# GPUs/goVideoCompressor

Hardware: AMD Instinct MI355X
Metric: encoded frames/sec (whole node), 1080p30->H.264 CRF23 (higher is better)
Workload: dtype uint8 (8-bit 4:2:0 samples, int32 transforms)

## Files before the change

csrc/kernels/encode_inter.hip:

```cpp
#include "h264_trellis.h"
#include "mb_row.h"

namespace mivc {
namespace gpu {

using h264::MbHeader;

struct InterArgs {
  Geom g;
  const uint8_t *src_y, *src_u, *src_v;
  const uint8_t *ref_y, *ref_u, *ref_v;
  uint8_t *rec_y, *rec_u, *rec_v;
  const uint8_t* pred_y;
  const int16_t* mv;
  const int16_t* mv8;
  const int* me_cost;
  const int* intra_cost;
  const int* qp;
  const int8_t* aq;
  int chroma_qp_offset;
  MbHeader* hdr;
  int16_t* coef;
  uint8_t* nz;
  uint8_t* intra_flag;
  int* intra_count;
  const uint8_t *ref1_u, *ref1_v;
  int bmode;
  int w1[4];
  int t8;
  const uint8_t* refs_u[4];
  const uint8_t* refs_v[4];
  const int8_t* mref;
  const int* wp;
  int trellis;
  float trellis_lambda;
  const SlotRoute* rt;
  int nbuf;
  uint8_t* qp_flags;
};


__device__ __forceinline__ int wp_sample(int p, int w, int o, int d) {
  return h264::clip1((d >= 1 ? ((p * w + (1 << (d - 1))) >> d) : p * w) + o);
}


__device__ __forceinline__ void chroma_mc4x4(const uint8_t* refc, int cw, int CH, int px0, int py0, int mvx, int mvy,
                                             int (&pv)[4][4]) {
  const int xf = mvx & 7, yf = mvy & 7;
  const int xi = px0 + (mvx >> 3), yi = py0 + (mvy >> 3);
  int rw[5][5];
  if (xi >= 0 && xi + 8 <= cw && yi >= 0 && yi + 5 <= CH) {
#pragma unroll
    for (int r = 0; r < 5; ++r) {
      const uint8_t* row = refc + static_cast<size_t>(yi + r) * cw;
      const int a = xi & ~3;
      const uint32_t w0 = *reinterpret_cast<const uint32_t*>(row + a), w1 = *reinterpret_cast<const uint32_t*>(row + a + 4);
      const uint32_t w4 = __builtin_amdgcn_alignbyte(w1, w0, xi & 3), w5 = row[xi + 4];
#pragma unroll
      for (int c = 0; c < 4; ++c) rw[r][c] = __builtin_amdgcn_ubfe(w4, 8 * c, 8);
      rw[r][4] = w5;
    }
  } else {
#pragma unroll
    for (int r = 0; r < 5; ++r) {
      const uint8_t* row = refc + static_cast<size_t>(clampi(yi + r, 0, CH - 1)) * cw;
#pragma unroll
      for (int c = 0; c < 5; ++c) rw[r][c] = row[clampi(xi + c, 0, cw - 1)];
    }
  }
  const int wA = (8 - xf) * (8 - yf), wB = xf * (8 - yf), wC = (8 - xf) * yf, wD = xf * yf;
#pragma unroll
  for (int y = 0; y < 4; ++y)
#pragma unroll
    for (int x = 0; x < 4; ++x)
      pv[y][x] = (wA * rw[y][x] + wB * rw[y][x + 1] + wC * rw[y + 1][x] + wD * rw[y + 1][x + 1] + 32) >> 6;
}

__device__ __forceinline__ int decimate_score(const int* scan, int start) {
  int score = 0, last = start - 1;
  bool big = false;
#pragma unroll
  for (int i = 0; i < 16; ++i) {
    if (i < start) continue;
    const int v = scan[i];
    const bool nzv = v != 0;
    big |= v > 1 || v < -1;
    const int run = i - last - 1;
    const int t = run == 0 ? 3 : (run <= 2 ? 2 : (run <= 5 ? 1 : 0));
    score += nzv ? t : 0;
    last = nzv ? i : last;
  }
  return big ? 9 : score;
}

__device__ __forceinline__ uint32_t ld4(const uint8_t* row, int x) {
  const int a = x & ~3;
  const uint32_t w0 = *reinterpret_cast<const uint32_t*>(row + a), w1 = *reinterpret_cast<const uint32_t*>(row + a + 4);
  return __builtin_amdgcn_alignbyte(w1, w0, x & 3);
}

__global__ __launch_bounds__(64) __attribute__((amdgpu_waves_per_eu(4, 8))) void encode_inter_mb(InterArgs a) {
  const Geom& g = a.g;
  const int lane = threadIdx.x, q = lane >> 4, l = lane & 15;
  const int nmb = g.nmb();
  int ux, slot;
  xcd_unit_slot(ux, slot);
  if (!route_active(a.rt, slot, a.bmode ? SK_B : SK_P)) return;
  const size_t rcur = route_index(a.rt, a.nbuf, slot, RO_CUR);
  const int W = g.W, cw = g.cw(), CH = g.ch();
  const int mb0 = ux * kMbsPerWave, mx0 = mb0 % g.wmb, my0 = mb0 / g.wmb;
  auto locate = [&](int qi, int& mx, int& my, size_t& o, bool& work, int& qp) {
    const bool live = mb0 + qi < nmb;
    const int d = live ? qi : nmb - 1 - mb0;
    mx = mx0 + d;
    my = my0;
#pragma unroll
    for (int i = 0; i < 3; ++i) {
      const bool wrap = mx >= g.wmb;
      mx -= wrap ? g.wmb : 0;
      my += wrap ? 1 : 0;
    }
    o = static_cast<size_t>(slot) * nmb + mb0 + d;
    work = live && !(a.intra_cost[o] < a.me_cost[o]);
    qp = clampi(a.qp[slot] + (a.aq ? a.aq[o] : 0), 0, 51);
    return live;
  };

  __shared__ uint32_t s_px[kMbsPerWave][2][16][4];
  __shared__ int s_d8[kMbsPerWave][4][64];

  auto store_levels = [](int16_t* dst, const int* v) {
    uint32_t w[8];
#pragma unroll
    for (int i = 0; i < 8; ++i) w[i] = (static_cast<uint32_t>(v[2 * i]) & 0xFFFFu) | (static_cast<uint32_t>(v[2 * i + 1]) << 16);
    reinterpret_cast<uint4*>(dst)[0] = make_uint4(w[0], w[1], w[2], w[3]);
    reinterpret_cast<uint4*>(dst)[1] = make_uint4(w[4], w[5], w[6], w[7]);
  };

  int lv[16];
  int res[16];
  uint32_t prw[4];
  uint64_t luma_any = 0;

  {
    int mx, my, qp;
    size_t o;
    bool work;
    const bool live = locate(q, mx, my, o, work, qp);
    MbHeader* h = a.hdr + o;
    int16_t* coef = a.coef + o * h264::kCoefPerMb;
    if (live && !work && l == 0) {
      a.intra_flag[o] = 1;
      atomicAdd(a.intra_count + slot, 1);
      h->kind = h264::MBK_I16x16;
    }
    const int X0 = mx * 16, Y0 = my * 16;
    const int lbx = (((l >> 2) & 1) * 2 + (l & 1)) * 4, lby = (((l >> 3) & 1) * 2 + ((l >> 1) & 1)) * 4;
    const int k = l & 3, ox = lbx & 4, oy = lby & 4;
    int* dd = s_d8[q][l >> 2];

    int score = 0;
    if (work) {
      const uint8_t* srcy = a.src_y + slot * g.ysize() + static_cast<size_t>(Y0 + lby) * W + X0 + lbx;
      const uint8_t* pred = a.pred_y + o * 256 + lby * 16 + lbx;
      uint32_t sw[4];
#pragma unroll
      for (int y = 0; y < 4; ++y) {
        prw[y] = *reinterpret_cast<const uint32_t*>(pred + y * 16);
        sw[y] = *reinterpret_cast<const uint32_t*>(srcy + static_cast<size_t>(y) * W);
      }
      if (a.wp && !a.bmode && !(a.mref && a.mref[o])) {
        const int* wt = a.wp + slot * 8;
        const int w = wt[0], wo = wt[1], d = wt[2];
        if (w != (1 << d) || wo != 0) {
#pragma unroll
          for (int y = 0; y < 4; ++y) {
            int v4[4];
#pragma unroll
            for (int x = 0; x < 4; ++x) v4[x] = wp_sample(static_cast<int>(__builtin_amdgcn_ubfe(prw[y], 8 * x, 8)), w, wo, d);
            prw[y] = pack4_u8(v4);
          }
        }
      }
#pragma unroll
      for (int y = 0; y < 4; ++y)
#pragma unroll
        for (int x = 0; x < 4; ++x)
          res[y * 4 + x] = static_cast<int>(__builtin_amdgcn_ubfe(sw[y], 8 * x, 8)) -
                           static_cast<int>(__builtin_amdgcn_ubfe(prw[y], 8 * x, 8));
      h264::forward_core4x4(res);
      int mf[3];
#pragma unroll
      for (int c = 0; c < 3; ++c) mf[c] = h264::kQuantMF[qp % 6][c];
      const int qbits = 15 + qp / 6;
      if (a.trellis) {
        trellis_lite4x4(res, lv, mf, qbits, trellis_lambda4(a.trellis_lambda, qp));
      } else {
#pragma unroll
        for (int r = 0; r < 16; ++r) lv[r] = h264::quant_coef(res[r], mf[h264::kPosClass[r]], qbits, 11);
      }
      int scan[16];
#pragma unroll
      for (int i = 0; i < 16; ++i) scan[i] = lv[h264::kZigzag4x4[i]];
      score = decimate_score(scan, 0);
      if (a.t8) {
#pragma unroll
        for (int y = 0; y < 4; ++y) {
          s_px[q][0][lby + y][lbx >> 2] = sw[y];
          s_px[q][1][lby + y][lbx >> 2] = prw[y];
        }
      }
    }
    const int score8 = sum4(score), score16 = sum16(score);
    const bool keep4 = score8 >= 4 && score16 >= 6;

    bool use8 = false, keep8 = false;
    uint64_t use8_wave = 0;
    if (a.t8) {
      wave_sync();
      const uint64_t try_wave = __ballot(keep4);
      if (try_wave) {
        const bool mine = ((try_wave >> (16 * q)) & 0xFFFFu) != 0;
        int satd = 0;
        if (mine) {
          int r2[16];
#pragma unroll
          for (int y = 0; y < 4; ++y) {
            const uint32_t sv = s_px[q][0][lby + y][lbx >> 2], pv = s_px[q][1][lby + y][lbx >> 2];
#pragma unroll
            for (int x = 0; x < 4; ++x) {
              r2[y * 4 + x] = static_cast<int>(__builtin_amdgcn_ubfe(sv, 8 * x, 8)) -
                              static_cast<int>(__builtin_amdgcn_ubfe(pv, 8 * x, 8));
              dd[(oy + y) * 8 + ox + x] = r2[y * 4 + x];
            }
          }
          satd = h264::satd4x4(r2);
        }
        const int col = l, grp = q;
        mfma_i32x4 sop, pop;
        {
          const int cm = col >> 2, b8 = col & 3, r0 = (b8 >> 1) * 8 + 2 * grp, c0 = (b8 & 1) * 2;
#pragma unroll
          for (int sp = 0; sp < 2; ++sp) {
            mfma_i32x4& op = sp ? pop : sop;
            op[0] = static_cast<int>(s_px[cm][sp][r0][c0] ^ 0x80808080u);
            op[1] = static_cast<int>(s_px[cm][sp][r0][c0 + 1] ^ 0x80808080u);
            op[2] = static_cast<int>(s_px[cm][sp][r0 + 1][c0] ^ 0x80808080u);
            op[3] = static_cast<int>(s_px[cm][sp][r0 + 1][c0 + 1] ^ 0x80808080u);
          }
        }
        mfma_i32x4 hp, hn;
#pragma unroll
        for (int j = 0; j < 4; ++j) {
          uint32_t w = 0;
#pragma unroll
          for (int b = 0; b < 4; ++b) w |= ((__builtin_popcount(col & (4 * j + b)) & 1) ? 0xFFu : 0x01u) << (8 * b);
          hp[j] = static_cast<int>(w);
          hn[j] = static_cast<int>(w ^ 0xFEFEFEFEu);
        }
        int sa = 0;
#pragma unroll
        for (int t = 0; t < 4; ++t) {
          const bool neg = __builtin_popcount(t & grp) & 1;
          mfma_i32x4 d = __builtin_amdgcn_mfma_i32_16x16x64_i8(neg ? hn : hp, sop, mfma_i32x4{0, 0, 0, 0}, 0, 0, 0);
          d = __builtin_amdgcn_mfma_i32_16x16x64_i8(neg ? hp : hn, pop, d, 0, 0, 0);
          sa += abs(d[0]) + abs(d[1]) + abs(d[2]) + abs(d[3]);
        }
        sa = sum_row_groups(sa);
        const int sa8d = __shfl(sum4((sa + 2) >> 2), 4 * q, 64);
        const int satd16 = sum16(satd);
        use8 = mine && sa8d < satd16;
        use8_wave = __ballot(use8);
        wave_sync();
        if (use8_wave) {
          if (use8) {
            dct8_pass(dd + (2 * k) * 8, 1);
            dct8_pass(dd + (2 * k + 1) * 8, 1);
          }
          wave_sync();
          if (use8) {
            dct8_pass(dd + 2 * k, 8);
            dct8_pass(dd + 2 * k + 1, 8);
          }
          wave_sync();
          const int qbits8 = 16 + qp / 6;
          const int m = qp % 6;
          if (a.trellis >= 2) {
            float z[16];
            int nzc = 0;
            if (use8) {
              const float inv = exp2f(-static_cast<float>(qbits8));
#pragma unroll
              for (int i = 0; i < 16; ++i) {
                const int pos = kZz8[k * 16 + i];
                const int mf8 = kQuant8MF[m][pos8(pos & 7, pos >> 3)];
                z[i] = static_cast<float>(dd[pos]) * static_cast<float>(mf8) * inv;
                nzc |= h264::quant_coef(dd[pos], mf8, qbits8, 11) != 0;
              }
            }
            const int nz1 = quad_bcast<1>(nzc), nz2 = quad_bcast<2>(nzc), nz3 = quad_bcast<3>(nzc);
            const bool later = (k < 1 && nz1) || (k < 2 && nz2) || (k < 3 && nz3);
            if (use8) trellis_lite8_chunk(z, lv, a.trellis_lambda * 0.136f, later);
          } else if (use8) {
#pragma unroll
            for (int i = 0; i < 16; ++i) {
              const int pos = kZz8[k * 16 + i];
              lv[i] = h264::quant_coef(dd[pos], kQuant8MF[m][pos8(pos & 7, pos >> 3)], qbits8, 11);
            }
          }
          int lastnz = -1, firstnz = -1, inner = 0, big = 0;
          if (use8) {
#pragma unroll
            for (int i = 0; i < 16; ++i) {
              const int idx = k * 16 + i;
              const int v = lv[i];
              const bool nzv = v != 0;
              big |= v > 1 || v < -1;
              const int run = idx - lastnz - 1;
              inner += (nzv && firstnz >= 0) ? (run <= 3 ? 3 : (run <= 11 ? 2 : (run <= 23 ? 1 : 0))) : 0;
              firstnz = (nzv && firstnz < 0) ? idx : firstnz;
              lastnz = nzv ? idx : lastnz;
            }
          }
          const int l0 = quad_bcast<0>(lastnz), l1 = quad_bcast<1>(lastnz), l2 = quad_bcast<2>(lastnz);
          const int prev = max(k > 0 ? l0 : -1, max(k > 1 ? l1 : -1, k > 2 ? l2 : -1));
          const int run0 = firstnz - prev - 1;
          const int sc = inner + (firstnz >= 0 ? (run0 <= 3 ? 3 : (run0 <= 11 ? 2 : (run0 <= 23 ? 1 : 0))) : 0);
          const int big8 = sum4(big), sc8 = sum4(sc);
          const int scb = big8 ? 9 : sc8;
          const int total8 = sum16(k == 0 ? scb : 0);
          keep8 = use8 && scb >= 4 && total8 >= 6;
        }
      }
    }

    bool any = false;
    if (use8_wave) {
      if (use8) {
#pragma unroll
        for (int i = 0; i < 16; ++i) lv[i] = keep8 ? lv[i] : 0;
        store_levels(coef + h264::COEF_LUMA + l * 16, lv);
        const int m = qp % 6, q6 = qp / 6;
#pragma unroll
        for (int i = 0; i < 16; ++i) {
          const int pos = kZz8[k * 16 + i];
          const int ls = 16 * kNorm8[m][pos8(pos & 7, pos >> 3)];
          const int c = lv[i];
          dd[pos] = q6 >= 6 ? (c * ls) << (q6 - 6) : (c * ls + (1 << (5 - q6))) >> (6 - q6);
        }
      }
      wave_sync();
      if (use8) {
        idct8_pass(dd + (2 * k) * 8, 1);
        idct8_pass(dd + (2 * k + 1) * 8, 1);
      }
      wave_sync();
      if (use8) {
        idct8_pass(dd + 2 * k, 8);
        idct8_pass(dd + 2 * k + 1, 8);
      }
      wave_sync();
      if (use8) {
        any = keep8;
#pragma unroll
        for (int y = 0; y < 4; ++y)
#pragma unroll
          for (int x = 0; x < 4; ++x) res[y * 4 + x] = (dd[(oy + y) * 8 + ox + x] + 32) >> 6;
      }
    }
    if (work && !use8) {
      int sv[16];
#pragma unroll
      for (int i = 0; i < 16; ++i) {
        sv[i] = keep4 ? lv[h264::kZigzag4x4[i]] : 0;
        any |= sv[i] != 0;
      }
      store_levels(coef + h264::COEF_LUMA + l * 16, sv);
      int dv[3];
#pragma unroll
      for (int c = 0; c < 3; ++c) dv[c] = h264::kDequantV[qp % 6][c];
#pragma unroll
      for (int r = 0; r < 16; ++r) res[r] = keep4 ? (lv[r] * dv[h264::kPosClass[r]]) << (qp / 6) : 0;
      if (any) h264::inverse_core4x4(res);
    }
    const bool t8_coded = ((__ballot(keep8) >> (16 * q)) & 0xFFFFu) != 0;
    luma_any = __ballot(any);
    if (work) {
      uint8_t* recy = a.rec_y + rcur * g.ysize() + static_cast<size_t>(Y0 + lby) * W + X0 + lbx;
#pragma unroll
      for (int y = 0; y < 4; ++y) {
        int v4[4];
#pragma unroll
        for (int x = 0; x < 4; ++x)
          v4[x] = h264::clip1(static_cast<int>(__builtin_amdgcn_ubfe(prw[y], 8 * x, 8)) + (any ? res[y * 4 + x] : 0));
        *reinterpret_cast<uint32_t*>(recy + static_cast<size_t>(y) * W) = pack4_u8(v4);
      }
      a.nz[o * 16 + (lbx >> 2) + lby] = any;
      if (l < 2) reinterpret_cast<uint4*>(coef + h264::COEF_LUMA_DC)[l] = make_uint4(0, 0, 0, 0);
      if (l == 0) {
        h->qp = static_cast<int8_t>(qp);
        h->i16_mode = 0;
        h->chroma_mode = 0;
        h->flags = t8_coded ? h264::MBF_T8x8 : 0;
        a.intra_flag[o] = 0;
        if (!a.bmode) {
          const int mvx = a.mv[o * 2], mvy = a.mv[o * 2 + 1];
          const uint32_t mvw = (static_cast<uint32_t>(mvx) & 0xFFFFu) | (static_cast<uint32_t>(mvy) << 16);
          uint4 q4 = make_uint4(mvw, mvw, mvw, mvw);
          if (a.mv8) q4 = *reinterpret_cast<const uint4*>(a.mv8 + o * 8);
          h->kind = (q4.x == q4.y && q4.z == q4.w) ? (q4.x == q4.z ? h264::MBK_P16x16 : h264::MBK_P16x8)
                                                   : ((q4.x == q4.z && q4.y == q4.w) ? h264::MBK_P8x16 : h264::MBK_P8x8);
          uint4* mvp = reinterpret_cast<uint4*>(&h->mv[0][0][0]);
          mvp[0] = q4;
          const uint32_t r = a.mref ? static_cast<uint32_t>(a.mref[o]) * 0x01010101u : 0u;
          *reinterpret_cast<uint2*>(&h->ref[0][0]) = make_uint2(r, 0xFFFFFFFFu);
        }
      }
    }
  }

  {
    const int comp = (lane >> 2) & 1, cb = lane & 3;
    int mx, my, qpy;
    size_t o;
    bool work;
    const bool live = locate((lane >> 3) & 3, mx, my, o, work, qpy);
    work = work && lane < 32;
    const MbHeader* h = a.hdr + o;
    int16_t* coef = a.coef + o * h264::kCoefPerMb;
    const int qpc = h264::chroma_qp(qpy, a.chroma_qp_offset);
    const int cbx = (cb & 1) * 4, cby = (cb >> 1) * 4;
    int mfc[3], dvc[3];
    int dc = 0, score = 0;
    if (work) {
#pragma unroll
      for (int c = 0; c < 3; ++c) {
        mfc[c] = h264::kQuantMF[qpc % 6][c];
        dvc[c] = h264::kDequantV[qpc % 6][c];
      }
      const uint8_t* srcc = (comp == 0 ? a.src_u : a.src_v) + slot * g.csize();
      const int px0 = mx * 8 + cbx, py0 = my * 8 + cby;
      int pv[4][4];
      if (!a.bmode) {
        const int cmx = a.mv8 ? a.mv8[o * 8 + cb * 2] : a.mv[o * 2], cmy = a.mv8 ? a.mv8[o * 8 + cb * 2 + 1] : a.mv[o * 2 + 1];
        const int r = a.mref ? a.mref[o] : 0;
        chroma_mc4x4((comp == 0 ? a.refs_u[r] : a.refs_v[r]) + route_index(a.rt, a.nbuf, slot, RO_L0 + r) * g.csize(), cw,
                     CH, px0, py0, cmx, cmy, pv);
        if (a.wp && r == 0) {
          const int* wt = a.wp + slot * 8;
          const int w = wt[3 + 2 * comp], wo = wt[4 + 2 * comp], d = wt[7];
          if (w != (1 << d) || wo != 0) {
#pragma unroll
            for (int y = 0; y < 4; ++y)
#pragma unroll
              for (int x = 0; x < 4; ++x) pv[y][x] = wp_sample(pv[y][x], w, wo, d);
          }
        }
      } else {
        const int r0 = h->ref[0][cb];
        const bool u0 = r0 >= 0, u1 = h->ref[1][cb] >= 0;
        const int w1 = a.rt ? a.rt[slot].w1[r0 & 3] : a.w1[r0 & 3];
        int p1[4][4];
        if (u0) chroma_mc4x4((comp == 0 ? a.refs_u[r0 & 3] : a.refs_v[r0 & 3]) +
                                 route_index(a.rt, a.nbuf, slot, RO_L0 + (r0 & 3)) * g.csize(), cw, CH, px0, py0,
                             h->mv[0][cb][0], h->mv[0][cb][1], pv);
        if (u1) chroma_mc4x4((comp == 0 ? a.ref1_u : a.ref1_v) + route_index(a.rt, a.nbuf, slot, RO_L1) * g.csize(), cw,
                             CH, px0, py0,
                             h->mv[1][cb][0], h->mv[1][cb][1], p1);
#pragma unroll
        for (int y = 0; y < 4; ++y)
#pragma unroll
          for (int x = 0; x < 4; ++x)
            pv[y][x] = u0 ? (u1 ? h264::clip1((pv[y][x] * (64 - w1) + p1[y][x] * w1 + 32) >> 6) : pv[y][x]) : p1[y][x];
      }
      uint32_t sw[4];
#pragma unroll
      for (int y = 0; y < 4; ++y) sw[y] = *reinterpret_cast<const uint32_t*>(srcc + static_cast<size_t>(py0 + y) * cw + px0);
#pragma unroll
      for (int y = 0; y < 4; ++y) {
#pragma unroll
        for (int x = 0; x < 4; ++x) res[y * 4 + x] = static_cast<int>(__builtin_amdgcn_ubfe(sw[y], 8 * x, 8)) - pv[y][x];
        prw[y] = pack4_u8(pv[y]);
      }
      h264::forward_core4x4(res);
      dc = res[0];
      const int qbits = 15 + qpc / 6;
      if (a.trellis >= 2) {
        trellis_lite4x4(res, lv, mfc, qbits, trellis_lambda4(a.trellis_lambda, qpc), 1);
      } else {
#pragma unroll
        for (int r = 0; r < 16; ++r)
          lv[r] = r == 0 ? 0 : h264::quant_coef(res[r], mfc[h264::kPosClass[r]], qbits, 11);
      }
      int scan[16];
#pragma unroll
      for (int i = 0; i < 16; ++i) scan[i] = lv[h264::kZigzag4x4[i]];
      score = decimate_score(scan, 1);
    }
    const int d0 = quad_bcast<0>(dc), d1 = quad_bcast<1>(dc), d2 = quad_bcast<2>(dc), d3 = quad_bcast<3>(dc);
    const int score_c = sum4(score);
    const bool keep_ac = score_c >= 7;
    bool any_c = false;
    if (work) {
      const int f[4] = {d0 + d1 + d2 + d3, d0 - d1 + d2 - d3, d0 + d1 - d2 - d3, d0 - d1 - d2 + d3};
      int cl[4];
#pragma unroll
      for (int i = 0; i < 4; ++i) cl[i] = h264::quant_coef(f[i], mfc[0], 15 + qpc / 6 + 1, 11);
      int sv[16];
      bool any_ac = false;
#pragma unroll
      for (int i = 0; i < 16; ++i) {
        sv[i] = (keep_ac && i > 0) ? lv[h264::kZigzag4x4[i]] : 0;
        any_ac |= sv[i] != 0;
      }
      store_levels(coef + h264::COEF_CHROMA_AC + (comp * 4 + cb) * 16, sv);
      if (cb == 0) {
        auto p2 = [](int lo, int hi) { return (static_cast<uint32_t>(lo) & 0xFFFFu) | (static_cast<uint32_t>(hi) << 16); };
        *reinterpret_cast<uint2*>(coef + h264::COEF_CHROMA_DC + comp * 4) = make_uint2(p2(cl[0], cl[1]), p2(cl[2], cl[3]));
      }
      const int c0 = cl[0], c1 = cl[1], c2 = cl[2], c3 = cl[3];
      const int fcb = cb == 0 ? c0 + c1 + c2 + c3 : (cb == 1 ? c0 - c1 + c2 - c3 : (cb == 2 ? c0 + c1 - c2 - c3 : c0 - c1 - c2 + c3));
      const int ls = 16 * dvc[0];
#pragma unroll
      for (int r = 0; r < 16; ++r) res[r] = (keep_ac && r > 0) ? (lv[r] * dvc[h264::kPosClass[r]]) << (qpc / 6) : 0;
      res[0] = ((fcb * ls) << (qpc / 6)) >> 5;
      const bool any = any_ac || c0 || c1 || c2 || c3;
      any_c = any;
      if (any) h264::inverse_core4x4(res);
      uint8_t* recc = (comp == 0 ? a.rec_u : a.rec_v) + rcur * g.csize() + static_cast<size_t>(my * 8 + cby) * cw + mx * 8 + cbx;
#pragma unroll
      for (int y = 0; y < 4; ++y) {
        int v4[4];
#pragma unroll
        for (int x = 0; x < 4; ++x)
          v4[x] = h264::clip1(static_cast<int>(__builtin_amdgcn_ubfe(prw[y], 8 * x, 8)) + (any ? res[y * 4 + x] : 0));
        *reinterpret_cast<uint32_t*>(recc + static_cast<size_t>(y) * cw) = pack4_u8(v4);
      }
    }
    if (a.qp_flags) {
      const uint64_t chroma_any = __ballot(any_c);
      const int m = (lane >> 3) & 3;
      if (live && lane < 32 && (lane & 7) == 0)
        a.qp_flags[o] = !work ? 2 : ((((luma_any >> (16 * m)) & 0xFFFFu) | ((chroma_any >> (8 * m)) & 0xFFu)) != 0 ? 1 : 0);
    }
  }
}

}
}

using namespace mivc::gpu;

extern "C" void mivc_launch_encode_inter(int B, int wmb, int hmb, const uint8_t* src_y, const uint8_t* src_u,
                                         const uint8_t* src_v, const uint8_t* ref_y, const uint8_t* ref_u,
                                         const uint8_t* ref_v, uint8_t* rec_y, uint8_t* rec_u, uint8_t* rec_v,
                                         const uint8_t* pred_y, const int16_t* mv, const int* me_cost,
                                         const int* intra_cost, const int* qp, int chroma_qp_offset, void* hdr,
                                         int16_t* coef, uint8_t* nz, uint8_t* intra_flag, int* intra_count,
                                         const int8_t* aq, const uint8_t* ref1_u, const uint8_t* ref1_v, int bmode,
                                         int t8, const int16_t* mv8, void* stream, const int* w1, int nref,
                                         const uint8_t* const* xref_u, const uint8_t* const* xref_v,
                                         const int8_t* mref, const int* wp, int trellis, float trellis_lambda,
                                         const void* route, int nbuf, uint8_t* qp_flags) {
  InterArgs a;
  a.qp_flags = qp_flags;
  a.rt = static_cast<const SlotRoute*>(route);
  a.nbuf = nbuf;
  a.trellis = trellis;
  a.trellis_lambda = trellis_lambda;
  a.wp = bmode ? nullptr : wp;
  for (int r = 0; r < 4; ++r) {
    const int rr = r < nref ? r : 0;
    a.refs_u[r] = rr == 0 ? ref_u : xref_u[rr];
    a.refs_v[r] = rr == 0 ? ref_v : xref_v[rr];
  }
  a.mref = mref;
  for (int r = 0; r < 4; ++r) a.w1[r] = w1[r < nref ? r : 0];
  a.g = Geom{B, wmb, hmb, wmb * 16, hmb * 16};
  a.src_y = src_y;
  a.src_u = src_u;
  a.src_v = src_v;
  a.ref_y = ref_y;
  a.ref_u = ref_u;
  a.ref_v = ref_v;
  a.rec_y = rec_y;
  a.rec_u = rec_u;
  a.rec_v = rec_v;
  a.pred_y = pred_y;
  a.mv = mv;
  a.mv8 = bmode ? nullptr : mv8;
  a.me_cost = me_cost;
  a.intra_cost = intra_cost;
  a.qp = qp;
  a.chroma_qp_offset = chroma_qp_offset;
  a.hdr = static_cast<MbHeader*>(hdr);
  a.coef = coef;
  a.nz = nz;
  a.intra_flag = intra_flag;
  a.intra_count = intra_count;
  a.aq = aq;
  a.ref1_u = ref1_u;
  a.ref1_v = ref1_v;
  a.bmode = bmode;
  a.t8 = t8;
  hipLaunchKernelGGL(encode_inter_mb, dim3(mb_row_grid(wmb * hmb), B), dim3(64), 0, static_cast<hipStream_t>(stream), a);
}
```

csrc/kernels/mb_row.h:

```cpp
#pragma once
#include "kcommon.h"

namespace mivc {
namespace gpu {

constexpr int kMbsPerWave = 4;

inline int mb_row_grid(int nmb) { return (nmb + kMbsPerWave - 1) / kMbsPerWave; }

struct MbRow {
  int slot, mb;
  int lane;
  int row;
  size_t o;
  int mx, my;
  int bx4, by4;
  int X, Y;
  bool live;
};

__device__ __forceinline__ MbRow mb_row(const Geom& g, const SlotRoute* rt = nullptr, int kind = -1) {
  MbRow r;
  int unit;
  xcd_unit_slot(unit, r.slot);
  r.lane = threadIdx.x & 15;
  r.row = threadIdx.x >> 4;
  r.mb = unit * kMbsPerWave + r.row;
  r.live = route_active(rt, r.slot, kind) && r.mb < g.nmb();
  r.o = static_cast<size_t>(r.slot) * g.nmb() + r.mb;
  r.mx = r.mb % g.wmb;
  r.my = r.mb / g.wmb;
  r.bx4 = (r.lane & 3) * 4;
  r.by4 = (r.lane >> 2) * 4;
  r.X = r.mx * 16 + r.bx4;
  r.Y = r.my * 16 + r.by4;
  return r;
}

__device__ __forceinline__ void load_src4(const Geom& g, const MbRow& r, const uint8_t* src_y, uint32_t (&s)[4]) {
  const size_t yo = static_cast<size_t>(r.slot) * g.ysize();
#pragma unroll
  for (int y = 0; y < 4; ++y)
    s[y] = *reinterpret_cast<const uint32_t*>(src_y + yo + static_cast<size_t>(r.Y + y) * g.W + r.X);
}

__device__ __forceinline__ int mb_lambda(const int* qp, const int8_t* aq, int slot, size_t o) {
  return h264::kLambda[clampi(qp[slot] + (aq ? aq[o] : 0), 0, 51)];
}

__device__ __forceinline__ int row_satd(const uint32_t (&src)[4], const uint32_t (&pw)[4]) {
  return sum16(satd4x4_u8(src, pw));
}

__device__ __forceinline__ bool moved_nearby(const Geom& g, const MbRow& r, const uint8_t* chg, bool below_left) {
  const int mb = r.mb, mx = r.mx, my = r.my;
  bool any = chg[mb];
  if (mx > 0) any = any || chg[mb - 1] || (below_left && my + 1 < g.hmb && chg[mb + g.wmb - 1]);
  if (my > 0)
    any = any || chg[mb - g.wmb] || (mx + 1 < g.wmb && chg[mb - g.wmb + 1]) || (mx > 0 && chg[mb - g.wmb - 1]);
  return any;
}

}
}
```

Measured before the change: 15950.

## Split inter chroma encoding into its own kernel and pack chroma MC in u16 pairs

Chroma residual coding moves out of the luma inter kernel into a separate kernel that handles 8 macroblocks per wave. The old path used only 32 of 64 lanes for chroma, and the new kernel uses all 64. Chroma motion compensation now builds byte pairs with v_perm and runs the bilinear filter on packed 16-bit vectors, with a packed fast path for bipred averaging. The cost is a second kernel launch, a recomputation of macroblock location and QP, and a split qp_flags write: luma writes the flag first and chroma then sets it to 1, which relies on the two launches being ordered on the same stream.

```diff
diff --git a/csrc/kernels/encode_inter.hip b/csrc/kernels/encode_inter.hip
--- a/csrc/kernels/encode_inter.hip
+++ b/csrc/kernels/encode_inter.hip
@@ -45,36 +45,68 @@
 }
 
 
+typedef unsigned short v2u16 __attribute__((ext_vector_type(2)));
+__device__ __forceinline__ v2u16 as_v2u16(uint32_t x) { return __builtin_bit_cast(v2u16, x); }
+__device__ __forceinline__ uint32_t as_u32(v2u16 x) { return __builtin_bit_cast(uint32_t, x); }
+__device__ __forceinline__ v2u16 splat_u16(int v) {
+  return v2u16{static_cast<unsigned short>(v), static_cast<unsigned short>(v)};
+}
+__device__ __forceinline__ int pair_lo(uint32_t p) { return static_cast<int>(p & 0xFFFFu); }
+__device__ __forceinline__ int pair_hi(uint32_t p) { return static_cast<int>(p >> 16); }
+__device__ __forceinline__ uint32_t make_pair(int lo, int hi) {
+  return static_cast<uint32_t>(lo) | (static_cast<uint32_t>(hi) << 16);
+}
+__device__ __forceinline__ uint32_t pairs_to_u8x4(const uint32_t (&p)[2]) {
+  return __builtin_amdgcn_perm(p[1], p[0], 0x06040200u);
+}
+
 __device__ __forceinline__ void chroma_mc4x4(const uint8_t* refc, int cw, int CH, int px0, int py0, int mvx, int mvy,
-                                             int (&pv)[4][4]) {
+                                             uint32_t (&pp)[4][2]) {
   const int xf = mvx & 7, yf = mvy & 7;
   const int xi = px0 + (mvx >> 3), yi = py0 + (mvy >> 3);
-  int rw[5][5];
+  uint32_t ra[5][2], rb[5][2];
   if (xi >= 0 && xi + 8 <= cw && yi >= 0 && yi + 5 <= CH) {
+    const uint32_t s = static_cast<uint32_t>(xi & 3) * 0x00010001u;
+    const uint32_t sa0 = 0x0c010c00u + s, sa1 = 0x0c030c02u + s, sb0 = 0x0c020c01u + s, sb1 = 0x0c040c03u + s;
 #pragma unroll
     for (int r = 0; r < 5; ++r) {
       const uint8_t* row = refc + static_cast<size_t>(yi + r) * cw;
       const int a = xi & ~3;
       const uint32_t w0 = *reinterpret_cast<const uint32_t*>(row + a), w1 = *reinterpret_cast<const uint32_t*>(row + a + 4);
-      const uint32_t w4 = __builtin_amdgcn_alignbyte(w1, w0, xi & 3), w5 = row[xi + 4];
-#pragma unroll
-      for (int c = 0; c < 4; ++c) rw[r][c] = __builtin_amdgcn_ubfe(w4, 8 * c, 8);
-      rw[r][4] = w5;
+      ra[r][0] = __builtin_amdgcn_perm(w1, w0, sa0);
+      ra[r][1] = __builtin_amdgcn_perm(w1, w0, sa1);
+      rb[r][0] = __builtin_amdgcn_perm(w1, w0, sb0);
+      rb[r][1] = __builtin_amdgcn_perm(w1, w0, sb1);
     }
   } else {
 #pragma unroll
     for (int r = 0; r < 5; ++r) {
       const uint8_t* row = refc + static_cast<size_t>(clampi(yi + r, 0, CH - 1)) * cw;
-#pragma unroll
-      for (int c = 0; c < 5; ++c) rw[r][c] = row[clampi(xi + c, 0, cw - 1)];
-    }
-  }
-  const int wA = (8 - xf) * (8 - yf), wB = xf * (8 - yf), wC = (8 - xf) * yf, wD = xf * yf;
+      int c[5];
+#pragma unroll
+      for (int i = 0; i < 5; ++i) c[i] = row[clampi(xi + i, 0, cw - 1)];
+      ra[r][0] = make_pair(c[0], c[1]);
+      ra[r][1] = make_pair(c[2], c[3]);
+      rb[r][0] = make_pair(c[1], c[2]);
+      rb[r][1] = make_pair(c[3], c[4]);
+    }
+  }
+  const v2u16 wA = splat_u16((8 - xf) * (8 - yf)), wB = splat_u16(xf * (8 - yf)), wC = splat_u16((8 - xf) * yf),
+              wD = splat_u16(xf * yf), half = splat_u16(32);
 #pragma unroll
   for (int y = 0; y < 4; ++y)
 #pragma unroll
-    for (int x = 0; x < 4; ++x)
-      pv[y][x] = (wA * rw[y][x] + wB * rw[y][x + 1] + wC * rw[y + 1][x] + wD * rw[y + 1][x + 1] + 32) >> 6;
+    for (int h = 0; h < 2; ++h)
+      pp[y][h] = as_u32((half + wA * as_v2u16(ra[y][h]) + wB * as_v2u16(rb[y][h]) + wC * as_v2u16(ra[y + 1][h]) +
+                         wD * as_v2u16(rb[y + 1][h])) >> 6);
+}
+
+__device__ __forceinline__ void store_levels(int16_t* dst, const int* v) {
+  uint32_t w[8];
+#pragma unroll
+  for (int i = 0; i < 8; ++i) w[i] = (static_cast<uint32_t>(v[2 * i]) & 0xFFFFu) | (static_cast<uint32_t>(v[2 * i + 1]) << 16);
+  reinterpret_cast<uint4*>(dst)[0] = make_uint4(w[0], w[1], w[2], w[3]);
+  reinterpret_cast<uint4*>(dst)[1] = make_uint4(w[4], w[5], w[6], w[7]);
 }
 
 __device__ __forceinline__ int decimate_score(const int* scan, int start) {
@@ -108,46 +140,29 @@
   xcd_unit_slot(ux, slot);
   if (!route_active(a.rt, slot, a.bmode ? SK_B : SK_P)) return;
   const size_t rcur = route_index(a.rt, a.nbuf, slot, RO_CUR);
-  const int W = g.W, cw = g.cw(), CH = g.ch();
-  const int mb0 = ux * kMbsPerWave, mx0 = mb0 % g.wmb, my0 = mb0 / g.wmb;
-  auto locate = [&](int qi, int& mx, int& my, size_t& o, bool& work, int& qp) {
-    const bool live = mb0 + qi < nmb;
-    const int d = live ? qi : nmb - 1 - mb0;
-    mx = mx0 + d;
-    my = my0;
+  const int W = g.W;
+  const int mb0 = ux * kMbsPerWave;
+
+  __shared__ uint32_t s_px[kMbsPerWave][2][16][4];
+  __shared__ int s_d8[kMbsPerWave][4][64];
+
+  int lv[16];
+  int res[16];
+  uint32_t prw[4];
+
+  {
+    const bool live = mb0 + q < nmb;
+    const int d = live ? q : nmb - 1 - mb0;
+    int mx = mb0 % g.wmb + d, my = mb0 / g.wmb;
 #pragma unroll
     for (int i = 0; i < 3; ++i) {
       const bool wrap = mx >= g.wmb;
       mx -= wrap ? g.wmb : 0;
       my += wrap ? 1 : 0;
     }
-    o = static_cast<size_t>(slot) * nmb + mb0 + d;
-    work = live && !(a.intra_cost[o] < a.me_cost[o]);
-    qp = clampi(a.qp[slot] + (a.aq ? a.aq[o] : 0), 0, 51);
-    return live;
-  };
-
-  __shared__ uint32_t s_px[kMbsPerWave][2][16][4];
-  __shared__ int s_d8[kMbsPerWave][4][64];
-
-  auto store_levels = [](int16_t* dst, const int* v) {
-    uint32_t w[8];
-#pragma unroll
-    for (int i = 0; i < 8; ++i) w[i] = (static_cast<uint32_t>(v[2 * i]) & 0xFFFFu) | (static_cast<uint32_t>(v[2 * i + 1]) << 16);
-    reinterpret_cast<uint4*>(dst)[0] = make_uint4(w[0], w[1], w[2], w[3]);
-    reinterpret_cast<uint4*>(dst)[1] = make_uint4(w[4], w[5], w[6], w[7]);
-  };
-
-  int lv[16];
-  int res[16];
-  uint32_t prw[4];
-  uint64_t luma_any = 0;
-
-  {
-    int mx, my, qp;
-    size_t o;
-    bool work;
-    const bool live = locate(q, mx, my, o, work, qp);
+    const size_t o = static_cast<size_t>(slot) * nmb + mb0 + d;
+    const bool work = live && !(a.intra_cost[o] < a.me_cost[o]);
+    const int qp = clampi(a.qp[slot] + (a.aq ? a.aq[o] : 0), 0, 51);
     MbHeader* h = a.hdr + o;
     int16_t* coef = a.coef + o * h264::kCoefPerMb;
     if (live && !work && l == 0) {
@@ -385,7 +400,10 @@
       if (any) h264::inverse_core4x4(res);
     }
     const bool t8_coded = ((__ballot(keep8) >> (16 * q)) & 0xFFFFu) != 0;
-    luma_any = __ballot(any);
+    if (a.qp_flags) {
+      const uint64_t luma_any = __ballot(any);
+      if (live && l == 0) a.qp_flags[o] = !work ? 2 : (((luma_any >> (16 * q)) & 0xFFFFu) != 0 ? 1 : 0);
+    }
     if (work) {
       uint8_t* recy = a.rec_y + rcur * g.ysize() + static_cast<size_t>(Y0 + lby) * W + X0 + lbx;
 #pragma unroll
@@ -420,130 +438,164 @@
     }
   }
 
-  {
-    const int comp = (lane >> 2) & 1, cb = lane & 3;
-    int mx, my, qpy;
-    size_t o;
-    bool work;
-    const bool live = locate((lane >> 3) & 3, mx, my, o, work, qpy);
-    work = work && lane < 32;
-    const MbHeader* h = a.hdr + o;
-    int16_t* coef = a.coef + o * h264::kCoefPerMb;
-    const int qpc = h264::chroma_qp(qpy, a.chroma_qp_offset);
-    const int cbx = (cb & 1) * 4, cby = (cb >> 1) * 4;
-    int mfc[3], dvc[3];
-    int dc = 0, score = 0;
-    if (work) {
-#pragma unroll
-      for (int c = 0; c < 3; ++c) {
-        mfc[c] = h264::kQuantMF[qpc % 6][c];
-        dvc[c] = h264::kDequantV[qpc % 6][c];
-      }
-      const uint8_t* srcc = (comp == 0 ? a.src_u : a.src_v) + slot * g.csize();
-      const int px0 = mx * 8 + cbx, py0 = my * 8 + cby;
-      int pv[4][4];
-      if (!a.bmode) {
-        const int cmx = a.mv8 ? a.mv8[o * 8 + cb * 2] : a.mv[o * 2], cmy = a.mv8 ? a.mv8[o * 8 + cb * 2 + 1] : a.mv[o * 2 + 1];
-        const int r = a.mref ? a.mref[o] : 0;
-        chroma_mc4x4((comp == 0 ? a.refs_u[r] : a.refs_v[r]) + route_index(a.rt, a.nbuf, slot, RO_L0 + r) * g.csize(), cw,
-                     CH, px0, py0, cmx, cmy, pv);
-        if (a.wp && r == 0) {
-          const int* wt = a.wp + slot * 8;
-          const int w = wt[3 + 2 * comp], wo = wt[4 + 2 * comp], d = wt[7];
-          if (w != (1 << d) || wo != 0) {
-#pragma unroll
-            for (int y = 0; y < 4; ++y)
-#pragma unroll
-              for (int x = 0; x < 4; ++x) pv[y][x] = wp_sample(pv[y][x], w, wo, d);
-          }
-        }
+}
+
+__global__ __launch_bounds__(64) void encode_inter_chroma(InterArgs a) {
+  const Geom& g = a.g;
+  const int lane = threadIdx.x, m = lane >> 3, comp = (lane >> 2) & 1, cb = lane & 3;
+  const int nmb = g.nmb();
+  int ux, slot;
+  xcd_unit_slot(ux, slot);
+  if (!route_active(a.rt, slot, a.bmode ? SK_B : SK_P)) return;
+  const size_t rcur = route_index(a.rt, a.nbuf, slot, RO_CUR);
+  const int cw = g.cw(), CH = g.ch();
+  const int mb0 = ux * kMbsPerChromaWave;
+  const bool live = mb0 + m < nmb;
+  const int dm = live ? m : nmb - 1 - mb0;
+  int mx = mb0 % g.wmb + dm, my = mb0 / g.wmb;
+  while (__ballot(mx >= g.wmb)) {
+    const bool wrap = mx >= g.wmb;
+    mx -= wrap ? g.wmb : 0;
+    my += wrap ? 1 : 0;
+  }
+  const size_t o = static_cast<size_t>(slot) * nmb + mb0 + dm;
+  const bool work = live && !(a.intra_cost[o] < a.me_cost[o]);
+  const int qpc = h264::chroma_qp(clampi(a.qp[slot] + (a.aq ? a.aq[o] : 0), 0, 51), a.chroma_qp_offset);
+  const MbHeader* h = a.hdr + o;
+  int16_t* coef = a.coef + o * h264::kCoefPerMb;
+  const int cbx = (cb & 1) * 4, cby = (cb >> 1) * 4;
+
+  int lv[16];
+  int res[16];
+  uint32_t prw[4];
+  int mfc[3], dvc[3];
+  int dc = 0, score = 0;
+  if (work) {
+#pragma unroll
+    for (int c = 0; c < 3; ++c) {
+      mfc[c] = h264::kQuantMF[qpc % 6][c];
+      dvc[c] = h264::kDequantV[qpc % 6][c];
+    }
+    const uint8_t* srcc = (comp == 0 ? a.src_u : a.src_v) + slot * g.csize();
+    const int px0 = mx * 8 + cbx, py0 = my * 8 + cby;
+    uint32_t pp[4][2];
+    if (!a.bmode) {
+      const int cmx = a.mv8 ? a.mv8[o * 8 + cb * 2] : a.mv[o * 2], cmy = a.mv8 ? a.mv8[o * 8 + cb * 2 + 1] : a.mv[o * 2 + 1];
+      const int r = a.mref ? a.mref[o] : 0;
+      chroma_mc4x4((comp == 0 ? a.refs_u[r] : a.refs_v[r]) + route_index(a.rt, a.nbuf, slot, RO_L0 + r) * g.csize(), cw,
+                   CH, px0, py0, cmx, cmy, pp);
+      if (a.wp && r == 0) {
+        const int* wt = a.wp + slot * 8;
+        const int w = wt[3 + 2 * comp], wo = wt[4 + 2 * comp], d = wt[7];
+        if (w != (1 << d) || wo != 0) {
+#pragma unroll
+          for (int y = 0; y < 4; ++y)
+#pragma unroll
+            for (int hh = 0; hh < 2; ++hh)
+              pp[y][hh] = make_pair(wp_sample(pair_lo(pp[y][hh]), w, wo, d), wp_sample(pair_hi(pp[y][hh]), w, wo, d));
+        }
+      }
+    } else {
+      const int r0 = h->ref[0][cb];
+      const bool u0 = r0 >= 0, u1 = h->ref[1][cb] >= 0;
+      const int w1 = a.rt ? a.rt[slot].w1[r0 & 3] : a.w1[r0 & 3];
+      uint32_t p1[4][2];
+      if (u0) chroma_mc4x4((comp == 0 ? a.refs_u[r0 & 3] : a.refs_v[r0 & 3]) +
+                               route_index(a.rt, a.nbuf, slot, RO_L0 + (r0 & 3)) * g.csize(), cw, CH, px0, py0,
+                           h->mv[0][cb][0], h->mv[0][cb][1], pp);
+      if (u1) chroma_mc4x4((comp == 0 ? a.ref1_u : a.ref1_v) + route_index(a.rt, a.nbuf, slot, RO_L1) * g.csize(), cw,
+                           CH, px0, py0,
+                           h->mv[1][cb][0], h->mv[1][cb][1], p1);
+      const bool bi = u0 && u1;
+      if (__ballot(bi && (w1 < 0 || w1 > 64)) == 0) {
+        const v2u16 k0 = splat_u16(64 - w1), k1 = splat_u16(w1), half = splat_u16(32);
+#pragma unroll
+        for (int y = 0; y < 4; ++y)
+#pragma unroll
+          for (int hh = 0; hh < 2; ++hh) {
+            const uint32_t b2 = as_u32((half + as_v2u16(pp[y][hh]) * k0 + as_v2u16(p1[y][hh]) * k1) >> 6);
+            pp[y][hh] = u0 ? (u1 ? b2 : pp[y][hh]) : p1[y][hh];
+          }
       } else {
-        const int r0 = h->ref[0][cb];
-        const bool u0 = r0 >= 0, u1 = h->ref[1][cb] >= 0;
-        const int w1 = a.rt ? a.rt[slot].w1[r0 & 3] : a.w1[r0 & 3];
-        int p1[4][4];
-        if (u0) chroma_mc4x4((comp == 0 ? a.refs_u[r0 & 3] : a.refs_v[r0 & 3]) +
-                                 route_index(a.rt, a.nbuf, slot, RO_L0 + (r0 & 3)) * g.csize(), cw, CH, px0, py0,
-                             h->mv[0][cb][0], h->mv[0][cb][1], pv);
-        if (u1) chroma_mc4x4((comp == 0 ? a.ref1_u : a.ref1_v) + route_index(a.rt, a.nbuf, slot, RO_L1) * g.csize(), cw,
-                             CH, px0, py0,
-                             h->mv[1][cb][0], h->mv[1][cb][1], p1);
 #pragma unroll
         for (int y = 0; y < 4; ++y)
 #pragma unroll
-          for (int x = 0; x < 4; ++x)
-            pv[y][x] = u0 ? (u1 ? h264::clip1((pv[y][x] * (64 - w1) + p1[y][x] * w1 + 32) >> 6) : pv[y][x]) : p1[y][x];
-      }
-      uint32_t sw[4];
-#pragma unroll
-      for (int y = 0; y < 4; ++y) sw[y] = *reinterpret_cast<const uint32_t*>(srcc + static_cast<size_t>(py0 + y) * cw + px0);
-#pragma unroll
-      for (int y = 0; y < 4; ++y) {
-#pragma unroll
-        for (int x = 0; x < 4; ++x) res[y * 4 + x] = static_cast<int>(__builtin_amdgcn_ubfe(sw[y], 8 * x, 8)) - pv[y][x];
-        prw[y] = pack4_u8(pv[y]);
-      }
-      h264::forward_core4x4(res);
-      dc = res[0];
-      const int qbits = 15 + qpc / 6;
-      if (a.trellis >= 2) {
-        trellis_lite4x4(res, lv, mfc, qbits, trellis_lambda4(a.trellis_lambda, qpc), 1);
-      } else {
-#pragma unroll
-        for (int r = 0; r < 16; ++r)
-          lv[r] = r == 0 ? 0 : h264::quant_coef(res[r], mfc[h264::kPosClass[r]], qbits, 11);
-      }
-      int scan[16];
-#pragma unroll
-      for (int i = 0; i < 16; ++i) scan[i] = lv[h264::kZigzag4x4[i]];
-      score = decimate_score(scan, 1);
-    }
-    const int d0 = quad_bcast<0>(dc), d1 = quad_bcast<1>(dc), d2 = quad_bcast<2>(dc), d3 = quad_bcast<3>(dc);
-    const int score_c = sum4(score);
-    const bool keep_ac = score_c >= 7;
-    bool any_c = false;
-    if (work) {
-      const int f[4] = {d0 + d1 + d2 + d3, d0 - d1 + d2 - d3, d0 + d1 - d2 - d3, d0 - d1 - d2 + d3};
-      int cl[4];
-#pragma unroll
-      for (int i = 0; i < 4; ++i) cl[i] = h264::quant_coef(f[i], mfc[0], 15 + qpc / 6 + 1, 11);
-      int sv[16];
-      bool any_ac = false;
-#pragma unroll
-      for (int i = 0; i < 16; ++i) {
-        sv[i] = (keep_ac && i > 0) ? lv[h264::kZigzag4x4[i]] : 0;
-        any_ac |= sv[i] != 0;
-      }
-      store_levels(coef + h264::COEF_CHROMA_AC + (comp * 4 + cb) * 16, sv);
-      if (cb == 0) {
-        auto p2 = [](int lo, int hi) { return (static_cast<uint32_t>(lo) & 0xFFFFu) | (static_cast<uint32_t>(hi) << 16); };
-        *reinterpret_cast<uint2*>(coef + h264::COEF_CHROMA_DC + comp * 4) = make_uint2(p2(cl[0], cl[1]), p2(cl[2], cl[3]));
-      }
-      const int c0 = cl[0], c1 = cl[1], c2 = cl[2], c3 = cl[3];
-      const int fcb = cb == 0 ? c0 + c1 + c2 + c3 : (cb == 1 ? c0 - c1 + c2 - c3 : (cb == 2 ? c0 + c1 - c2 - c3 : c0 - c1 - c2 + c3));
-      const int ls = 16 * dvc[0];
-#pragma unroll
-      for (int r = 0; r < 16; ++r) res[r] = (keep_ac && r > 0) ? (lv[r] * dvc[h264::kPosClass[r]]) << (qpc / 6) : 0;
-      res[0] = ((fcb * ls) << (qpc / 6)) >> 5;
-      const bool any = any_ac || c0 || c1 || c2 || c3;
-      any_c = any;
-      if (any) h264::inverse_core4x4(res);
-      uint8_t* recc = (comp == 0 ? a.rec_u : a.rec_v) + rcur * g.csize() + static_cast<size_t>(my * 8 + cby) * cw + mx * 8 + cbx;
-#pragma unroll
-      for (int y = 0; y < 4; ++y) {
-        int v4[4];
-#pragma unroll
-        for (int x = 0; x < 4; ++x)
-          v4[x] = h264::clip1(static_cast<int>(__builtin_amdgcn_ubfe(prw[y], 8 * x, 8)) + (any ? res[y * 4 + x] : 0));
-        *reinterpret_cast<uint32_t*>(recc + static_cast<size_t>(y) * cw) = pack4_u8(v4);
-      }
-    }
-    if (a.qp_flags) {
-      const uint64_t chroma_any = __ballot(any_c);
-      const int m = (lane >> 3) & 3;
-      if (live && lane < 32 && (lane & 7) == 0)
-        a.qp_flags[o] = !work ? 2 : ((((luma_any >> (16 * m)) & 0xFFFFu) | ((chroma_any >> (8 * m)) & 0xFFu)) != 0 ? 1 : 0);
-    }
+          for (int hh = 0; hh < 2; ++hh) {
+            const int lo = h264::clip1((pair_lo(pp[y][hh]) * (64 - w1) + pair_lo(p1[y][hh]) * w1 + 32) >> 6);
+            const int hi = h264::clip1((pair_hi(pp[y][hh]) * (64 - w1) + pair_hi(p1[y][hh]) * w1 + 32) >> 6);
+            pp[y][hh] = u0 ? (u1 ? make_pair(lo, hi) : pp[y][hh]) : p1[y][hh];
+          }
+      }
+    }
+    uint32_t sw[4];
+#pragma unroll
+    for (int y = 0; y < 4; ++y) sw[y] = *reinterpret_cast<const uint32_t*>(srcc + static_cast<size_t>(py0 + y) * cw + px0);
+#pragma unroll
+    for (int y = 0; y < 4; ++y) {
+#pragma unroll
+      for (int x = 0; x < 4; ++x)
+        res[y * 4 + x] = static_cast<int>(__builtin_amdgcn_ubfe(sw[y], 8 * x, 8)) -
+                         ((x & 1) ? pair_hi(pp[y][x >> 1]) : pair_lo(pp[y][x >> 1]));
+      prw[y] = pairs_to_u8x4(pp[y]);
+    }
+    h264::forward_core4x4(res);
+    dc = res[0];
+    const int qbits = 15 + qpc / 6;
+    if (a.trellis >= 2) {
+      trellis_lite4x4(res, lv, mfc, qbits, trellis_lambda4(a.trellis_lambda, qpc), 1);
+    } else {
+#pragma unroll
+      for (int r = 0; r < 16; ++r)
+        lv[r] = r == 0 ? 0 : h264::quant_coef(res[r], mfc[h264::kPosClass[r]], qbits, 11);
+    }
+    int scan[16];
+#pragma unroll
+    for (int i = 0; i < 16; ++i) scan[i] = lv[h264::kZigzag4x4[i]];
+    score = decimate_score(scan, 1);
+  }
+  const int d0 = quad_bcast<0>(dc), d1 = quad_bcast<1>(dc), d2 = quad_bcast<2>(dc), d3 = quad_bcast<3>(dc);
+  const int score_c = sum4(score);
+  const bool keep_ac = score_c >= 7;
+  bool any_c = false;
+  if (work) {
+    const int f[4] = {d0 + d1 + d2 + d3, d0 - d1 + d2 - d3, d0 + d1 - d2 - d3, d0 - d1 - d2 + d3};
+    int cl[4];
+#pragma unroll
+    for (int i = 0; i < 4; ++i) cl[i] = h264::quant_coef(f[i], mfc[0], 15 + qpc / 6 + 1, 11);
+    int sv[16];
+    bool any_ac = false;
+#pragma unroll
+    for (int i = 0; i < 16; ++i) {
+      sv[i] = (keep_ac && i > 0) ? lv[h264::kZigzag4x4[i]] : 0;
+      any_ac |= sv[i] != 0;
+    }
+    store_levels(coef + h264::COEF_CHROMA_AC + (comp * 4 + cb) * 16, sv);
+    if (cb == 0) {
+      auto p2 = [](int lo, int hi) { return (static_cast<uint32_t>(lo) & 0xFFFFu) | (static_cast<uint32_t>(hi) << 16); };
+      *reinterpret_cast<uint2*>(coef + h264::COEF_CHROMA_DC + comp * 4) = make_uint2(p2(cl[0], cl[1]), p2(cl[2], cl[3]));
+    }
+    const int c0 = cl[0], c1 = cl[1], c2 = cl[2], c3 = cl[3];
+    const int fcb = cb == 0 ? c0 + c1 + c2 + c3 : (cb == 1 ? c0 - c1 + c2 - c3 : (cb == 2 ? c0 + c1 - c2 - c3 : c0 - c1 - c2 + c3));
+    const int ls = 16 * dvc[0];
+#pragma unroll
+    for (int r = 0; r < 16; ++r) res[r] = (keep_ac && r > 0) ? (lv[r] * dvc[h264::kPosClass[r]]) << (qpc / 6) : 0;
+    res[0] = ((fcb * ls) << (qpc / 6)) >> 5;
+    const bool any = any_ac || c0 || c1 || c2 || c3;
+    any_c = any;
+    if (any) h264::inverse_core4x4(res);
+    uint8_t* recc = (comp == 0 ? a.rec_u : a.rec_v) + rcur * g.csize() + static_cast<size_t>(my * 8 + cby) * cw + mx * 8 + cbx;
+#pragma unroll
+    for (int y = 0; y < 4; ++y) {
+      int v4[4];
+#pragma unroll
+      for (int x = 0; x < 4; ++x)
+        v4[x] = h264::clip1(static_cast<int>(__builtin_amdgcn_ubfe(prw[y], 8 * x, 8)) + (any ? res[y * 4 + x] : 0));
+      *reinterpret_cast<uint32_t*>(recc + static_cast<size_t>(y) * cw) = pack4_u8(v4);
+    }
+  }
+  if (a.qp_flags) {
+    const uint64_t chroma_any = __ballot(any_c);
+    if (work && (lane & 7) == 0 && ((chroma_any >> (8 * m)) & 0xFFu) != 0) a.qp_flags[o] = 1;
   }
 }
 
@@ -605,4 +657,5 @@
   a.bmode = bmode;
   a.t8 = t8;
   hipLaunchKernelGGL(encode_inter_mb, dim3(mb_row_grid(wmb * hmb), B), dim3(64), 0, static_cast<hipStream_t>(stream), a);
-}
+  hipLaunchKernelGGL(encode_inter_chroma, dim3(chroma_wave_grid(wmb * hmb), B), dim3(64), 0, static_cast<hipStream_t>(stream), a);
+}
diff --git a/csrc/kernels/mb_row.h b/csrc/kernels/mb_row.h
--- a/csrc/kernels/mb_row.h
+++ b/csrc/kernels/mb_row.h
@@ -7,6 +7,9 @@
 constexpr int kMbsPerWave = 4;
 
 inline int mb_row_grid(int nmb) { return (nmb + kMbsPerWave - 1) / kMbsPerWave; }
+
+constexpr int kMbsPerChromaWave = 8;
+inline int chroma_wave_grid(int nmb) { return (nmb + kMbsPerChromaWave - 1) / kMbsPerChromaWave; }
 
 struct MbRow {
   int slot, mb;
```

Result: faster. 16430 (median of 6 runs) (+3.0%).
